# kocvara/Loraine.jl

Hardware: AMD Instinct MI355X
Metric: ms/IP-iteration (Schur assembly + solve), dense SDP n=2000 m=4000 (lower is better)
Workload: dtype f64; 1 GPU; C4 synthetic dense SDP, matrix side 2000, 4000 constraints, kit=0 (assembly + Cholesky + predictor/corrector solves); msz=2000, nvar=4000, seed=20250614, parallelism=1 GPU

## Files before the change

### include/loraine_hip.h

```cpp
#ifndef LORAINE_HIP_H
#define LORAINE_HIP_H

#include <stdint.h>

#ifdef __cplusplus
extern "C" {
#endif

typedef struct lrn_ctx lrn_ctx;

int lrn_create(lrn_ctx** out, int device);
int lrn_destroy(lrn_ctx* ctx);
const char* lrn_last_error(lrn_ctx* ctx);
int lrn_version(void);
int lrn_device_count(void);

int lrn_upload_model(lrn_ctx* ctx, int nlmi, int nvar, const int64_t* msizes,
                     const int64_t* const* AA_colptr, const int64_t* const* AA_rowval,
                     const double* const* AA_nzval,
                     const int64_t* const* B_colptr, const int64_t* const* B_rowval,
                     const double* const* B_nzval,
                     const int64_t* sigmaA, const int64_t* qA,
                     int nlin, const int64_t* Clin_colptr, const int64_t* Clin_rowval,
                     const double* Clin_nzval);
// ... 66 lines not shown
int lrn_comm_allreduce(lrn_ctx* ctx, double* buf, int64_t count, int op);

int lrn_get_timing(lrn_ctx* ctx, const char* key, double* ms);
int64_t lrn_get_count(lrn_ctx* ctx, const char* key);
int lrn_mfma_f64_peak(lrn_ctx* ctx, double* tflops);
int lrn_xcc_probe(lrn_ctx* ctx, int nx, int nz, int hold_us, int32_t* out);
int lrn_hbm_copy_peak(lrn_ctx* ctx, int64_t bytes, double* gbps);

int lrn_dbg_gemm(lrn_ctx* ctx, int transA, int transB, int M, int N, int K, double alpha,
                 const double* A, int lda, const double* B, int ldb, double beta, double* C,
                 int ldc, int flags, int ksplit);
int lrn_dbg_product(lrn_ctx* ctx, int kind, int n, const double* A, const double* Bm, double alpha, double a, int tri,
                    double* out0, double* out1, double* scalar);
int lrn_dbg_gemm_plan(int transA, int transB, int M, int N, int K, int lda, int ldb, double beta, int ldc, int flags,
                      int ksplit, int* out6);
int lrn_dbg_schur_chol_plan(int msz, int nd, int rank, int world, int64_t pcap_hint, const int* opts6, int64_t* out10, int* kb,
                            int* ke, int* weights, double* shares3);
int lrn_dbg_mfma_probe(lrn_ctx* ctx, const double* A16x4, const double* B4x16, double* D16x16);
int lrn_dbg_potrf(lrn_ctx* ctx, int n, double* A, int* info);
int lrn_dbg_potrs(lrn_ctx* ctx, int n, const double* A, const double* b, double* x, int* info);
int lrn_dbg_trsm(lrn_ctx* ctx, int n, int nrhs, int trans, const double* A, double* B, int* info);
int lrn_dbg_svd_jacobi(lrn_ctx* ctx, int n, const double* A, double* U_sigma, double* V,
                       double* sigma, int* sweeps);

#ifdef __cplusplus
}
#endif
#endif
```

### loraine.jl_amd/_capi.py

```python
import ctypes as C
import os
import shutil
import subprocess
import sys

import numpy as np

_HERE = os.path.dirname(os.path.abspath(__file__))
LIB_PATH = os.path.join(_HERE, "libloraine_hip.so")

c_ctx = C.c_void_p
PD = C.POINTER(C.c_double)
PI64 = C.POINTER(C.c_int64)
PI = C.POINTER(C.c_int)
PPD = C.POINTER(C.c_void_p)

SIGNATURES = {
    "lrn_create": (C.c_int, [C.POINTER(c_ctx), C.c_int]),
    "lrn_destroy": (C.c_int, [c_ctx]),
    "lrn_last_error": (C.c_char_p, [c_ctx]),
    "lrn_version": (C.c_int, []),
    "lrn_device_count": (C.c_int, []),
    "lrn_upload_model": (C.c_int, [c_ctx, C.c_int, C.c_int, C.c_void_p, PPD, PPD, PPD, PPD, PPD, PPD,
                                   C.c_void_p, C.c_void_p, C.c_int, C.c_void_p, C.c_void_p, C.c_void_p]),
# ... 47 lines not shown
    "lrn_dbg_get_block": (C.c_int, [c_ctx, C.c_int, C.c_char_p, C.c_void_p, PI]),
    "lrn_dbg_tridiag_eig": (C.c_int, [C.c_int, C.c_void_p, C.c_void_p, C.c_int, C.c_void_p, C.c_double, PD, PI64]),
    "lrn_dbg_eigmin": (C.c_int, [c_ctx, C.c_int, C.c_void_p, PD, PI]),
    "lrn_dbg_lanczos": (C.c_int, [c_ctx, C.c_int, C.c_int, C.c_void_p, C.c_void_p, C.c_void_p, PD, PD, PI]),
    "lrn_get_timing": (C.c_int, [c_ctx, C.c_char_p, PD]),
    "lrn_get_count": (C.c_int64, [c_ctx, C.c_char_p]),
    "lrn_mfma_f64_peak": (C.c_int, [c_ctx, PD]),
    "lrn_hbm_copy_peak": (C.c_int, [c_ctx, C.c_int64, PD]),
    "lrn_xcc_probe": (C.c_int, [c_ctx, C.c_int, C.c_int, C.c_int, C.c_void_p]),
    "lrn_dbg_gemm": (C.c_int, [c_ctx, C.c_int, C.c_int, C.c_int, C.c_int, C.c_int, C.c_double, C.c_void_p,
                               C.c_int, C.c_void_p, C.c_int, C.c_double, C.c_void_p, C.c_int, C.c_int, C.c_int]),
    "lrn_dbg_product": (C.c_int, [c_ctx, C.c_int, C.c_int, C.c_void_p, C.c_void_p, C.c_double, C.c_double, C.c_int,
                                  C.c_void_p, C.c_void_p, PD]),
    "lrn_dbg_gemm_plan": (C.c_int, [C.c_int, C.c_int, C.c_int, C.c_int, C.c_int, C.c_int, C.c_int, C.c_double, C.c_int,
                                    C.c_int, C.c_int, PI]),
    "lrn_dbg_schur_chol_plan": (C.c_int, [C.c_int, C.c_int, C.c_int, C.c_int, C.c_int64, PI, PI64, PI, PI, PI, PD]),
    "lrn_dbg_mfma_probe": (C.c_int, [c_ctx, C.c_void_p, C.c_void_p, C.c_void_p]),
    "lrn_dbg_potrf": (C.c_int, [c_ctx, C.c_int, C.c_void_p, PI]),
    "lrn_dbg_potrs": (C.c_int, [c_ctx, C.c_int, C.c_void_p, C.c_void_p, C.c_void_p, PI]),
    "lrn_dbg_trsm": (C.c_int, [c_ctx, C.c_int, C.c_int, C.c_int, C.c_void_p, C.c_void_p, PI]),
    "lrn_dbg_svd_jacobi": (C.c_int, [c_ctx, C.c_int, C.c_void_p, C.c_void_p, C.c_void_p, C.c_void_p, PI]),
}

GEMM_TRI_LOWER, GEMM_TRI_UPPER, GEMM_OFFDIAG_X2, GEMM_SQUARE, GEMM_KSEG_TRI, GEMM_SMALL_TILE = 1, 2, 4, 8, 16, 32
GEMM_KFROM_N, GEMM_KFROM_M, GEMM_KTO_N, GEMM_KTO_M, GEMM_C_MIRROR, GEMM_DYN_MASKS = 64, 128, 1024, 2048, 4096, 131072

_lib = None


class LoraineHipError(RuntimeError):
# ... 58 lines not shown
```

### loraine.jl_amd/csrc/api.hip

```cpp
#include <cstring>

#include "../../include/loraine_hip.h"
#include "ctx.h"
#include "ops.h"
#include "schur_plan.h"

using namespace lrn;

void lrn_free_model(lrn_ctx* c);
namespace lrn {
void prec_free(lrn_ctx* c);
}

extern "C" {

int lrn_version(void) { return 102; }

int lrn_device_count(void) {
  int n = 0;
  if (hipGetDeviceCount(&n) != hipSuccess) {
    (void)hipGetLastError();
    return 0;
  }
  return n;
// ... 63 lines not shown
  if (!c || !key) return LRN_ERR_ARG;
  if (!strcmp(key, "dense_threshold")) c->opt.dense_threshold = value;
  else if (!strcmp(key, "profile")) c->profile = value != 0.0;
  else if (!strcmp(key, "t_batch")) { c->opt.t_batch = (long)value; for (auto& b : c->lmi) b.t_cap = b.p_cap = 0; }
  else if (!strcmp(key, "p_batch")) { c->opt.p_batch = (long)value; for (auto& b : c->lmi) b.t_cap = b.p_cap = 0; }
  else if (!strcmp(key, "prec_eig")) c->opt.prec_eig = (int)value;
  else if (!strcmp(key, "pivot_boost")) c->opt.pivot_boost = value;
  else if (!strcmp(key, "schur_chol")) c->opt.schur_chol = (int)value;
  else if (!strcmp(key, "schur_plan")) c->opt.schur_plan = (int)value;
  else if (!strcmp(key, "gemm3_ksplit")) c->opt.gemm3_ksplit = (int)value;
  else if (!strcmp(key, "gemm_no_skip")) c->opt.gemm_no_skip = (int)value;
  else if (!strcmp(key, "gemm_dyn_masks")) c->opt.gemm_dyn_masks = (int)value;
  else if (!strcmp(key, "gemm1_diag")) c->opt.gemm1_diag = (int)value;
  else if (!strcmp(key, "gemm_lab")) c->opt.gemm_lab = (int)value & 127;
  else if (!strcmp(key, "gemm3_sched")) c->opt.gemm3_sched = (int)value;
  else if (!strcmp(key, "gemm3_tile")) c->opt.gemm3_tile = (int)value;
  else if (!strcmp(key, "gemm3_strip")) c->opt.gemm3_strip = (int)value;
  else if (!strcmp(key, "gemm3_stagger")) c->opt.gemm3_stagger = (int)value;
  else if (!strcmp(key, "jacobi_wgs")) c->opt.jacobi_wgs = (int)value;
  else if (!strcmp(key, "jacobi_block")) c->opt.jacobi_block = (int)value;
  else if (!strcmp(key, "jacobi_inner")) c->opt.jacobi_inner = (int)value;
  else if (!strcmp(key, "pair_lanes")) c->opt.pair_lanes = (int)value;
  else if (!strcmp(key, "matvec_sparse")) c->opt.matvec_sparse = (int)value;
  else if (!strcmp(key, "prec_dense")) c->opt.prec_dense = (int)value;
  else if (!strcmp(key, "wmw_pattern_min")) c->opt.wmw_pattern_min = std::max(2, (int)value);
  else if (!strcmp(key, "profile_symv")) c->opt.profile_symv = (int)value;
  else if (!strcmp(key, "profile_ops")) c->opt.profile_ops = (int)value;
  else if (!strcmp(key, "matvec_h")) { c->opt.matvec_h = (int)value; c->hop_version = -1; }
  else if (!strcmp(key, "comm_fail_ensure")) lrn::comm_inject_ensure_failure(c);
  else if (!strcmp(key, "pcg_lookahead")) c->opt.pcg_lookahead = std::max(0, std::min(8, (int)value));
// ... 464 lines not shown
    if (flags & GEMM_KSEG_TRI) {
      int ld = 1;
      while ((long)(ld + 1) * (ld + 1) <= K) ++ld;
      g.kseg_ld = ld; g.kseg_cols = ld;
    }
  } else {
    g.sCm = 1; g.sCn = ldc; g.beta = beta;
  }
  GemmPlanInfo info;
  const int rc = gemm_plan_info(g, &info);
  const int v[6] = {info.kernel, info.tile, info.grid_x, info.grid_z, info.dyn_lds, info.slabs};
  for (int i = 0; i < 6; ++i) out6[i] = v[i];
  return rc;
}

int lrn_dbg_schur_chol_plan(int msz, int nd, int rank, int world, int64_t pcap_hint, const int* opts6, int64_t* out10, int* kb,
                            int* ke, int* weights, double* shares3) {
  if (!opts6 || !out10 || !kb || !ke || !weights || !shares3 || msz < 1 || nd < 1 || world < 1 || rank < 0 || rank >= world)
    return LRN_ERR_ARG;
  CholPlanOpts o;
  o.p_batch = opts6[0]; o.gemm3_tile = opts6[1]; o.gemm3_ksplit = opts6[2];
  o.gemm3_sched = opts6[3]; o.gemm3_strip = opts6[4]; o.gemm_no_skip = opts6[5];
  const CholPlan p = plan_chol(msz, nd, rank, world, (long)pcap_hint, o);
  const int64_t v[10] = {p.idle ? -1 : p.c0, p.idle ? -1 : p.c1, p.p_elems, p.ldp, p.P_cap, p.t160 ? 160 : 128,
                         p.ncls,             p.cls[0],           p.cls[1],  p.nslab};
  for (int i = 0; i < 10; ++i) out10[i] = v[i];
  for (int s = 0; s < p.nslab; ++s) { kb[s] = p.kb[s]; ke[s] = p.ke[s]; weights[s] = (int)p.sw.w[s]; }
  shares3[0] = p.gemm1_share; shares3[1] = p.gemm2_share; shares3[2] = p.gemm3_share;
  return LRN_OK;
}
// ... 79 lines not shown
```

### loraine.jl_amd/csrc/ctx.h

```cpp
#pragma once
#include <map>

#include "chol.h"
#include "lrn_common.h"

namespace lrn { struct Prec; struct Comm; }

struct LmiBlock {
  int msz = 0;
  long nent = 0;
  std::vector<int> sigma;
  std::vector<int> ipos;
  std::vector<long> nnz;
  int qA = 0;
  int nd = 0;
  int q_wave = 0;
  int npos_nz = 0;
  long p_cap = 0, t_cap = 0;
  lrn::DBuf ent_ptr;
  lrn::DBuf ent_r, ent_c;
  lrn::DBuf ent_v;
  lrn::DBuf Adense;
  enum DenseRoute { DENSE_SCALAR = 0, DENSE_STREAM, DENSE_TRI };
  DenseRoute dense_route = DENSE_SCALAR;
// ... 47 lines not shown

struct LrnOptions {
  double dense_threshold = -1.0;
  long t_batch = 0, p_batch = 0;
  int prec_eig = 0;
  double pivot_boost = 1e-12;
  int schur_chol = -1;
  int schur_plan = -1;
  int gemm3_ksplit = 0;
  int gemm_dyn_masks = 0;
  int gemm_lab = 0;
  int gemm1_diag = 1;
  int gemm_no_skip = 0;
  int gemm3_sched = 1;
  int gemm3_strip = 1;
  int gemm3_tile = 0;
  int gemm3_stagger = 0;
  int jacobi_inner = 0;
  int jacobi_wgs = 0;
  int jacobi_block = 0;
  int jacobi_cross = 1;
  int prepw_streams = 1;
  int lz_resident = 1;
  int eigmin_pair = 2;
  double jacobi_early = 3e-8;
  bool jacobi_warm = true;
  int shard_passes = 1;
  int prec_inv = -1;
  int nt_mode = 1;
  double ns_l0 = 2e-3;
// ... 144 lines not shown
```

### loraine.jl_amd/csrc/gemm_f64.hip

```cpp
#include "lrn_common.h"

#include <algorithm>
#include <cstdlib>
#include <map>
#include <mutex>
#include <tuple>
#include <type_traits>
#include <utility>
#include <vector>

namespace lrn {

static constexpr int BK = 16;
static constexpr int MAX_KSPLIT = 64;

struct GemmParams {
  GemmDesc d;
  int tilesM, tilesN;
  int kchunk;
  int kcols[MAX_KSPLIT + 1];
  int kcols2[MAX_KSPLIT + 1];
  const int2* tile_list;
  const int2* tile_list2;
  int n1, n2;
  int m_org = 0, n_org = 0;
};

#define MFMA_F64_ROW(lane, r) (((lane) >> 4) + 4 * (r))
#define LRN_MFMA_INPLACE(c, a, b) asm volatile("v_mfma_f64_16x16x4_f64 %0, %1, %2, %0" : "+v"(c) : "v"(a), "v"(b))
#define LRN_MFMA_DRAIN() asm volatile("s_nop 15\n\ts_nop 15\n\ts_nop 15" ::: "memory")

template <int BM, bool KC>
__device__ __forceinline__ int lds_idx(int m, int k) {
  return KC ? (m * (BK + 2) + k) : (k * (BM + 16) + m);
}

template <int BM, int BN, bool AKC, bool BKC, bool KSEG, bool EPI>
__global__ __launch_bounds__(256, 2) void gemm_f64_kernel(GemmParams p) {
  constexpr int TM = BM / 32, TN = BN / 32;
// ... 218 lines not shown
  return bkc ? gemm_f64_kernel<BT, BT, false, true, KSEG, EPI> : gemm_f64_kernel<BT, BT, false, false, KSEG, EPI>;
}
template <int BT>
static GemmFn reg_kernel(const GemmDesc& d, bool epi) {
  if (d.flags & GEMM_KSEG_TRI) return reg_kernel<BT, true, false>(d);
  return epi ? reg_kernel<BT, false, true>(d) : reg_kernel<BT, false, false>(d);
}

template <bool EPI, bool DYN>
__global__ __launch_bounds__(256, 2) void gemm_f64_lds_kernel(GemmParams p) {
  constexpr int BM = 128, BN = 128, TM = 4, TN = 4;
  constexpr int LROW = BM + 16;
  constexpr int LA = BK * LROW;
  __shared__ double lds[2 * 2 * LA];
  const GemmDesc& d = p.d;
  int tm, tn;
  {
    int bid = blockIdx.x, nwg = gridDim.x;
    int q = nwg >> 3, r = nwg & 7, xcd = bid & 7;
    int swz = (xcd < r ? xcd * (q + 1) : r * (q + 1) + (xcd - r) * q) + (bid >> 3);
    if ((d.flags & (GEMM_KFROM_N | GEMM_KFROM_M | GEMM_KTO_N | GEMM_KTO_M)) && r == 0) {
      xcd = (xcd + (int)blockIdx.z) & 7;
      swz = xcd * q + (bid >> 3);
    }
    int2 tt = p.tile_list[swz];
    tm = tt.x;
    tn = tt.y;
  }
  if (tm < 0) return;
  const int bz = blockIdx.z;
  const double* Ag = d.A + (long)bz * d.bA;
  const double* Bg = d.B + (long)bz * d.bB;
  double* __restrict__ Cg = d.C + (long)bz * d.bC;
  const int t = threadIdx.x, lane = t & 63;
  const int w = __builtin_amdgcn_readfirstlane(t >> 6);
  const int wm = w & 1, wn = w >> 1;
  const int m0 = tm * BM, n0 = tn * BN;
  const int lda = (int)d.sAk, ldb = (int)d.sBk;
  const int Me = d.M + (d.M & 1) <= lda ? d.M + (d.M & 1) : d.M;
  const int Ne = d.N + (d.N & 1) <= ldb ? d.N + (d.N & 1) : d.N;
  const unsigned bytesA = (unsigned)(((long)(d.K - 1) * lda + Me) * 8);
  const unsigned bytesB = (unsigned)(((long)(d.K - 1) * ldb + Ne) * 8);
  __amdgpu_buffer_rsrc_t ra = __builtin_amdgcn_make_buffer_rsrc((void*)Ag, 0, bytesA, 0x00020000);
  __amdgpu_buffer_rsrc_t rb = __builtin_amdgcn_make_buffer_rsrc((void*)Bg, 0, bytesB, 0x00020000);
  const int ma = m0 + 2 * lane, nb = n0 + 2 * lane;
// ... 359 lines not shown
#pragma unroll
      for (int r = 0; r < 4; ++r) {
        const int m = m0 + wm * 32 + i * 16 + MFMA_F64_ROW(lane, r);
        const int n = n0 + wn * 32 + j * 16 + fr;
        if (m < d.M && n < d.N) Cg[(long)m * d.sCm + n] = d.alpha * acc[i][j][r];
      }
  if (trace && t == 0) trace[7] = wall_clock64();
}

template <bool FLAT, int TBM, int TBN>
__global__ __launch_bounds__(256, 2) void gemm_f64_kseg_lds_kernel(GemmParams p) {
  constexpr int BM = 32 * TBM, BN = 32 * TBN, TM = TBM, TN = TBN;
  constexpr int LA = BM * BK, LB = BN * BK;
  extern __shared__ double lds[];
  const GemmDesc& d = p.d;
  int tm, tn, ks, bz;
  if (p.n2 >= 0) {
    const int xcd = blockIdx.x & 7, l = blockIdx.x >> 3;
    const int q1 = p.n1 >> 3, q2 = p.n2 >> 3;
    int2 tt;
    if (l < d.ksplit * q1) { ks = l / q1; tt = p.tile_list[xcd * q1 + l % q1]; }
    else { const int l2 = l - d.ksplit * q1; ks = l2 / q2; tt = p.tile_list2[xcd * q2 + l2 % q2]; }
    tm = tt.x;
    tn = tt.y;
    bz = 0;
  } else {
    int bid = blockIdx.x, nwg = gridDim.x;
    int q = nwg >> 3, r = nwg & 7, xcd = bid & 7;
    int swz = (xcd < r ? xcd * (q + 1) : r * (q + 1) + (xcd - r) * q) + (bid >> 3);
    int2 tt = p.tile_list[swz];
    tm = tt.x;
    tn = tt.y;
    ks = blockIdx.z % d.ksplit;
    bz = blockIdx.z / d.ksplit;
  }
  if (tm < 0) return;
  const double* Ag = d.A + (long)bz * d.bA;
  const double* Bg = d.B + (long)bz * d.bB;
  double* __restrict__ Cg = d.C + (long)bz * d.bC + (long)ks * d.sCs;
  const int t = threadIdx.x, lane = t & 63;
  const int w = __builtin_amdgcn_readfirstlane(t >> 6);
  const int wm = w & 1, wn = w >> 1;
  const int m0 = p.m_org + tm * BM, n0 = p.n_org + tn * BN;
  const int lrow = lane >> 3, lpair = lane & 7;
  const double* pa[TBM];
  const double* pb[TBN];
#pragma unroll
  for (int j = 0; j < TBM; ++j) {
    int row = 8 * (w + 4 * j) + lrow;
    int src_pair = lpair ^ ((row >> 1) & 7);
// ... 160 lines not shown
enum GemmKernel : int {
  GK_NONE = 0,
  GK_REG64,
  GK_REG128,
  GK_LDS,
  GK_MID,
  GK_KSEG,
  GK_KFLAT128,
  GK_KFLAT160,
  GK_KFLAT_STRIP,
};

struct TileListKey {
  int tilesM, tilesN, tri, short_sel;
  bool edge_m, edge_n, diag;
  int n;
};

struct GemmPlan {
  GemmKernel kernel;
  int tile_m, tile_n;
  dim3 grid;
  unsigned dyn_lds;
  bool epi;
  int slabs;
  int nlists;
  TileListKey lists[2];
  GemmParams p;
};

static thread_local const char* tls_gemm_error = nullptr;
// ... 22 lines not shown
  const bool tri = d.flags & (GEMM_TRI_LOWER | GEMM_TRI_UPPER);
  return !epi && d.batch == 1 && d.beta == 0.0 && d.sAm == 1 && d.sBn == 1 && d.K >= 64 && d.sCn == 1 && d.sAk >= d.M &&
         d.sBk >= d.N && !(d.flags & ~(GEMM_SMALL_TILE | GEMM_TRI_LOWER | GEMM_TRI_UPPER)) &&
         (!tri || (d.M == d.N && d.ksplit > 1)) && (double)d.K * (double)std::max(d.sAk, d.sBk) * 8.0 < 2.0e9;
}

static bool tile_in_list(const TileListKey& k, int tm, int tn) {
  if (k.tri == GEMM_TRI_LOWER && tn > tm) return false;
  if (k.tri == GEMM_TRI_UPPER && tm > tn) return false;
  const bool shrt = (k.edge_m && tm == k.tilesM - 1) || (k.edge_n && tn == k.tilesN - 1) || (k.diag && tm == tn);
  return !((k.short_sel == 1 && shrt) || (k.short_sel == 2 && !shrt));
}

static TileListKey tile_list_key(int tilesM, int tilesN, int tri, int short_sel = 0, bool edge_m = false, bool edge_n = false,
                                 bool diag = false) {
  TileListKey k{tilesM, tilesN, tri & (GEMM_TRI_LOWER | GEMM_TRI_UPPER), short_sel, edge_m, edge_n, diag, 0};
  if (!k.tri && !short_sel) k.n = tilesM * tilesN;
  else
    for (int tn = 0; tn < tilesN; ++tn)
      for (int tm = 0; tm < tilesM; ++tm) k.n += tile_in_list(k, tm, tn);
  k.n = (k.n + 7) & ~7;
  return k;
}

static const int2* get_tile_list(const TileListKey& k) {
  static std::map<std::tuple<int, int, int>, int2*> cache[16];
  static std::mutex mu;
  std::lock_guard<std::mutex> lock(mu);
  int dev = 0;
  (void)hipGetDevice(&dev);
  auto& cm = cache[dev & 15];
  const std::tuple<int, int, int> key{k.tilesM, k.tilesN, k.tri | k.short_sel << 8 | k.edge_m << 12 | k.edge_n << 13 | k.diag << 14};
  auto it = cm.find(key);
  if (it != cm.end()) return it->second;
  std::vector<int2> v;
  const int GS = 8;
// ... 131 lines not shown
  }
  const bool kseg = d.flags & GEMM_KSEG_TRI;
  if (kseg && kseg_lds_path_ok(d)) return GK_KSEG;
  if (!kseg && !small && lds_path_ok(d)) return GK_LDS;
  if (!kseg && small && mid_path_ok(d, epi)) return GK_MID;
  return small ? GK_REG64 : GK_REG128;
}

static void plan_two_lists(GemmPlan* plan, int tilesM, int tilesN, int tri, bool em, bool en, bool dg) {
  GemmParams& p = plan->p;
  plan->nlists = 2;
  plan->lists[0] = tile_list_key(tilesM, tilesN, tri, 1, em, en, dg);
  plan->lists[1] = tile_list_key(tilesM, tilesN, tri, 2, em, en, dg);
  const bool only_short = plan->lists[0].n == 0;
  if (only_short) plan->lists[0] = plan->lists[1];
  p.n1 = plan->lists[0].n;
  p.n2 = only_short ? 0 : plan->lists[1].n;
}

static int plan_gemm(const GemmDesc& din, GemmPlan* plan, int slabs = 0) {
  *plan = GemmPlan{};
  plan->slabs = slabs > 0 ? slabs : auto_split_factor(din);
  GemmParams& p = plan->p;
  p.d = din;
  GemmDesc& d = p.d;
  if (plan->slabs > 1) {
    d.sCs = (long)din.M * din.N; d.ksplit = plan->slabs; d.beta = 0.0;
    d.flags |= GEMM_SMALL_TILE;
  }
  if (d.M <= 0 || d.N <= 0 || d.batch <= 0) return LRN_OK;
  if (!d.A || !d.B || (!d.C && plan->slabs == 1)) return gemm_fail(LRN_ERR_ARG, "gemm: null A, B or C");
  if (d.ksplit < 1) d.ksplit = 1;
// ... 11 lines not shown
      (!d.blk_w || d.blk_k < 1 || d.blk_k > 16 || (d.blk_k & (d.blk_k - 1)) || d.M % d.blk_k || d.N % d.blk_k ||
       d.ksplit != 1 || d.batch != 1 || kseg || kfrom || d.C2 ||
       (d.flags & (GEMM_SQUARE | GEMM_OFFDIAG_X2 | GEMM_C_PACKED | GEMM_C_MIRROR))))
    return gemm_fail(LRN_ERR_ARG, "gemm: GEMM_SQUARE_BLOCKSUM needs blk_w, blk_k in {1, 2, 4, 8, 16} dividing M and N, one "
                                  "unsplit, unbatched product and no other epilogue");
  if ((d.flags & GEMM_C_PACKED) && (d.pk_off & 15)) return gemm_fail(LRN_ERR_ARG, "gemm: GEMM_C_PACKED needs pk_off % 16 == 0 (block width of the packed layout)");
  if ((d.flags & GEMM_C_PACKED) && (!swapped || d.pk_m <= 0 || d.beta != 0.0)) return gemm_fail(LRN_ERR_ARG, "gemm: (d.flags & GEMM_C_PACKED) && (!swapped || d.pk_m <= 0 || d.beta != 0.0)");
  const bool small = want_small_tile(d, kseg, kfrom);
  const bool big = kflat && (d.flags & GEMM_TILE160);
  const int BMv = small ? 64 : (big ? 160 : 128);
  p.tilesM = (d.M + BMv - 1) / BMv;
  p.tilesN = (d.N + BMv - 1) / BMv;
  if (const int rc = plan_k_ranges(p); rc != LRN_OK) return rc;
  if (d.tile_class >= 4 && !kflat) return gemm_fail(LRN_ERR_ARG, "gemm: tile_class 4 / 5 are for the K-contiguous rank-k update");
  if (d.tile_class != 0 && small) return gemm_fail(LRN_ERR_ARG, "gemm: tile_class needs the 128 tile");
  p.n2 = -1;
  plan->epi = (d.flags & (GEMM_OFFDIAG_X2 | GEMM_SQUARE | GEMM_SQUARE_BLOCKSUM | GEMM_C_PACKED | GEMM_C_MIRROR)) || d.C2;
  plan->tile_m = plan->tile_n = BMv;
  const GemmKernel kernel = choose_kernel(d, small, plan->epi);
  const bool em = (d.M % BMv) != 0, en = (d.N % BMv) != 0, dg = (d.flags & (GEMM_DIAG_LOWER | GEMM_DIAG_UPPER)) != 0;
  if (d.tile_class == 3) {
    if (!kflat || d.batch != 1) return gemm_fail(LRN_ERR_ARG, "gemm: tile_class 3 is for the K-contiguous rank-k update");
    plan_two_lists(plan, p.tilesM, p.tilesN, trif, em, en, dg);
  } else if (d.tile_class == 4 || d.tile_class == 5) {
    const int rem = d.M % 128;
    if (d.batch != 1 || big || d.M != d.N || rem == 0 || rem > 32 || d.M < 288 || trif != GEMM_TRI_UPPER ||
        !(d.flags & GEMM_DIAG_UPPER) || (d.flags & GEMM_NO_SKIP))
      return gemm_fail(LRN_ERR_ARG, "gemm: tile_class 4 needs the symmetric K-contiguous update with M % 128 in (0, 32]");
    const int Mm = d.M - 128 - rem, tmain = Mm / 128;
    if (d.tile_class == 4) {
      d.M = d.N = Mm;
// ... 1 lines not shown
      plan_two_lists(plan, tmain, tmain, GEMM_TRI_UPPER, false, false, true);
    } else {
      d.flags &= ~(GEMM_TRI_LOWER | GEMM_TRI_UPPER | GEMM_DIAG_LOWER | GEMM_DIAG_UPPER);
      p.n_org = Mm;
      p.tilesM = tmain + 2; p.tilesN = 1;
      plan->tile_n = 160;
      plan->nlists = 1;
      plan->lists[0] = tile_list_key(tmain + 2, 1, 0);
    }
  } else {
    plan->nlists = 1;
    plan->lists[0] = tile_list_key(p.tilesM, p.tilesN, trif, d.tile_class, d.tile_class != 0 && em, d.tile_class != 0 && en,
                                   d.tile_class != 0 && dg);
  }
  if (plan->lists[0].n == 0) return LRN_OK;
  if (plan->nlists == 2) {
    const long wgs = 8L * d.ksplit * ((p.n1 >> 3) + (p.n2 >> 3));
    if (wgs > 0x7fffffffL) return gemm_fail(LRN_ERR_ARG, "gemm: grid too large");
    plan->grid = dim3((unsigned)wgs, 1, 1);
  } else {
    plan->grid = dim3(plan->lists[0].n, 1, d.batch * d.ksplit);
    if (plan->grid.z > 65535) return gemm_fail(LRN_ERR_ARG, "gemm: grid.z > 65535");
  }
  if (d.C2 && (d.M != d.N || d.batch != 1 || d.ksplit != 1 || kseg)) return gemm_fail(LRN_ERR_ARG, "gemm: C2 needs a square, unbatched, unsplit product");
  if (kernel == GK_KSEG) plan->dyn_lds = 2 * 2 * 128 * BK * 8;
  else if (kernel > GK_KSEG) plan->dyn_lds = 2 * (plan->tile_m + plan->tile_n) * BK * 8;
  else if (kernel == GK_LDS && (d.flags & (GEMM_LAB_ONE_WG | GEMM_DYN_MASKS)) == GEMM_LAB_ONE_WG) plan->dyn_lds = 24576;
  else if (kernel == GK_MID) {
    p.n1 = (trif ? p.tilesM * (p.tilesM + 1) / 2 : p.tilesM * p.tilesN) * d.ksplit;
    plan->grid = dim3((unsigned)((p.n1 + 7) & ~7), 1, 1);
  }
  plan->kernel = kernel;
  return LRN_OK;
// ... 101 lines not shown
    return LRN_OK;
  }
  if (out) { out->p = din.C; out->stride = 0; out->n = 1; }
  if (!slabs) return LRN_OK;
  const int tri = din.flags != GEMM_TRI_LOWER ? 0 : (std::labs(din.sCm) == 1 ? GEMM_TRI_LOWER : GEMM_TRI_UPPER);
  return reduce_slabs(st, slabs, (long)mn, plan.slabs, din.C, (long)mn, din.beta, tri, din.M);
}

int gemm(hipStream_t st, const GemmDesc& din) { return gemm_maybe_slabs(st, din, nullptr); }
int gemm_slabs(hipStream_t st, const GemmDesc& din, SlabSrc* out) { return gemm_maybe_slabs(st, din, out); }

int gemm_plan_info(const GemmDesc& d, GemmPlanInfo* info) {
  tls_gemm_error = nullptr;
  GemmPlan plan;
  const int rc = plan_gemm(d, &plan);
  *info = GemmPlanInfo{(int)plan.kernel, plan.tile_m, (int)plan.grid.x, (int)plan.grid.z, (int)plan.dyn_lds, plan.slabs};
  return rc;
}

template <bool TRI>
__global__ void reduce_slabs_kernel(const double* __restrict__ slabs, long stride, int nslab,
                                    double* __restrict__ out, long n, double beta, int tri, int ld) {
  long i = (long)blockIdx.x * blockDim.x + threadIdx.x;
  long step = (long)gridDim.x * blockDim.x;
  for (; i < n; i += step) {
    if (TRI) {
      const long r = (i % ld) >> 6, c = (i / ld) >> 6;
      if (tri == GEMM_TRI_LOWER ? r < c : r > c) continue;
    }
    double s = 0.0;
    for (int k = 0; k < nslab; ++k) s += slabs[(long)k * stride + i];
// ... 67 lines not shown
```

### loraine.jl_amd/csrc/lrn_common.h

```cpp
#pragma once
#include <hip/hip_runtime.h>

#include <cstdint>
#include <cstdio>
#include <cstring>
#include <string>
#include <vector>

#define LRN_OK 0
#define LRN_ERR_ARG (-1)
#define LRN_ERR_HIP (-2)
#define LRN_ERR_STATE (-3)
#define LRN_ERR_NOMEM (-4)

typedef double v4f64 __attribute__((ext_vector_type(4)));

namespace lrn {

__host__ __device__ inline int shard_owner(int blk, int world) {
  int r = blk % world;
  return ((blk / world) & 1) ? world - 1 - r : r;
}
__host__ __device__ inline int shard_global_block(int rank, int lb, int world) {
  return lb * world + ((lb & 1) ? world - 1 - rank : rank);
// ... 67 lines not shown
  long sCs = 0;
  int kseg_ld = 0, kseg_cols = 0;
  int pk_m = 0;
  long pk_cstride = 16;
  int pk_off = 0;
  long kflat_cstride = 16;
  const int* kflat_kb = nullptr;
  const int* kflat_ke = nullptr;
  long kflat_total = 0, kflat_diag = 0;
  int kflat_nsd = 0;
  int tile_class = 0;
  unsigned long long* lab_trace = nullptr;
  int kstagger = 0;
  const double* blk_w = nullptr;
  int blk_k = 0;
};

int gemm(hipStream_t st, const GemmDesc& d);
struct SlabSrc {
  const double* p = nullptr;
  long stride = 0;
  int n = 1;
};
__device__ __forceinline__ double slab_sum(const SlabSrc& s, long e) {
  double v = 0.0;
  for (int k = 0; k < s.n; ++k) v += s.p[(long)k * s.stride + e];
  return v;
}
int gemm_slabs(hipStream_t st, const GemmDesc& d, SlabSrc* out);
const char* gemm_last_error();
int reduce_slabs(hipStream_t st, const double* slabs, long stride, int nslab, double* out,
                 long n, double beta, int tri = 0, int ld = 0);
struct GemmPlanInfo { int kernel, tile, grid_x, grid_z, dyn_lds, slabs; };
int gemm_plan_info(const GemmDesc& d, GemmPlanInfo* info);
int mfma_f64_peak(hipStream_t st, double* tflops);
int mfma_f64_probe(hipStream_t st, const double* A16x4, const double* B4x16, double* D16x16);

}
```

### loraine.jl_amd/csrc/schur_dense.hip

```cpp
#include "ops.h"
#include "schur_plan.h"

namespace lrn {

static constexpr int TS = 128;
static constexpr int BK_CHUNK = 16;

__global__ __launch_bounds__(256) void dense_sparse_gather_kernel(
    const long* __restrict__ ptr, const int* __restrict__ er, const int* __restrict__ ec,
    const double* __restrict__ ev, const double* __restrict__ T, int msz, int s0, int ns, int p_lo,
    int p_end, const int* __restrict__ hidx, double* __restrict__ H, int ldh) {
  const int s = blockIdx.y;
  if (s >= ns) return;
  const int pj = p_lo + blockIdx.x * 256 + threadIdx.x;
  if (pj >= p_end) return;
  const double* Ts = T + (long)s * msz * msz;
  double acc = 0.0;
  for (long f = ptr[pj]; f < ptr[pj + 1]; ++f) {
    int p = er[f], q = ec[f];
    int tp = p / TS, tq = q / TS;
    double t;
    if (tp == tq) t = Ts[(long)p + (long)q * msz];
    else if (tp > tq) t = 0.5 * Ts[(long)p + (long)q * msz];
    else t = 0.5 * Ts[(long)q + (long)p * msz];
// ... 133 lines not shown
  return LRN_OK;
}

static int chol_lab12(const LrnOptions& o) {
  return (o.gemm_no_skip ? GEMM_NO_SKIP : 0) | (o.gemm_dyn_masks ? GEMM_DYN_MASKS : 0) | ((o.gemm_lab & 15) << 20);
}
static GemmDesc chol_gemm1(const lrn_ctx* c, const CholPlan& pl, int m, const double* Ad, const double* Ut, double* P, int a,
                           int nbat) {
  const long mm = (long)m * m, off = (long)pl.c0 + (long)pl.c0 * m;
  GemmDesc g1;
  g1.A = Ad + (long)a * mm + off; g1.sAm = 1; g1.sAk = m; g1.bA = mm;
  g1.B = Ut + off; g1.sBk = m; g1.sBn = 1; g1.bB = 0;
  g1.C = P; g1.sCm = pl.ldp; g1.sCn = 1; g1.bC = pl.p_elems;
  g1.M = g1.K = m - pl.c0; g1.N = pl.c1 - pl.c0; g1.batch = nbat;
  g1.flags = GEMM_TRI_LOWER | GEMM_KFROM_N | chol_lab12(c->opt) | (c->opt.gemm1_diag ? GEMM_DIAG_LOWER_Z : 0);
  if (c->opt.gemm_lab & 32) g1.bA = 0;
  if (c->opt.gemm_lab & 16) g1.flags &= ~GEMM_KFROM_N;
  return g1;
}
static GemmDesc chol_gemm2(const lrn_ctx* c, const CholPlan& pl, int m, const double* Ut, const double* P, double* T,
                           long cstride, int a, int nbat) {
  const long off = (long)pl.c0 + (long)pl.c0 * m;
  GemmDesc g2;
  g2.A = Ut + off; g2.sAm = 1; g2.sAk = m; g2.bA = 0;
  g2.B = P; g2.sBk = pl.ldp; g2.sBn = 1; g2.bB = pl.p_elems;
  g2.C = T + (long)a * 16; g2.sCm = 1; g2.sCn = m; g2.bC = 16;
  g2.pk_cstride = cstride;
  g2.M = g2.K = m - pl.c0; g2.N = pl.c1 - pl.c0; g2.batch = nbat;
  g2.flags = GEMM_TRI_LOWER | GEMM_KFROM_M | GEMM_C_PACKED | chol_lab12(c->opt);
  if (c->opt.gemm_lab & 32) g2.bB = 0;
  if (c->opt.gemm_lab & 16) g2.flags &= ~GEMM_KFROM_M;
  g2.pk_m = m;
  g2.pk_off = pl.c0;
  return g2;
}
static GemmDesc chol_gemm3(const lrn_ctx* c, const CholPlan& pl, int m, int nd, const double* T, long cstride, double* slabs) {
  GemmDesc g3;
  g3.A = T; g3.sAm = 16; g3.sAk = 1;
  g3.B = T; g3.sBk = 1; g3.sBn = 16;
  g3.kflat_cstride = cstride;
  g3.C = slabs; g3.sCm = 1; g3.sCn = nd;
  g3.M = nd; g3.N = nd;
  g3.flags = GEMM_TRI_LOWER | GEMM_KFLAT | GEMM_DIAG_LOWER | (c->opt.gemm_no_skip ? GEMM_NO_SKIP : 0) |
             (pl.t160 ? GEMM_TILE160 : 0) | ((c->opt.gemm_lab & 64) ? GEMM_LAB_SAME_CHUNK : 0);
  g3.kflat_total = packed_total_elems(m); g3.kflat_diag = packed_diag_elems(m); g3.kflat_nsd = 1;
  g3.kflat_kb = pl.kb; g3.kflat_ke = pl.ke;
  g3.kstagger = c->opt.gemm3_stagger;
  g3.ksplit = pl.nslab; g3.sCs = (long)nd * nd;
  return g3;
}

static int assemble_dense_chol(lrn_ctx* c, LmiBlock& b, long pcap_hint) {
  const int m = b.msz, nd = b.nd;
  CholPlanOpts po;
  po.p_batch = c->opt.p_batch; po.gemm3_tile = c->opt.gemm3_tile; po.gemm3_ksplit = c->opt.gemm3_ksplit;
  po.gemm3_sched = c->opt.gemm3_sched; po.gemm3_strip = c->opt.gemm3_strip; po.gemm_no_skip = c->opt.gemm_no_skip;
  const CholPlan pl = plan_chol(m, nd, c->rank, c->world, pcap_hint, po);
  c->timing["gemm1_share"] = pl.gemm1_share;
  c->timing["gemm2_share"] = pl.gemm2_share;
  c->timing["gemm3_share"] = pl.gemm3_share;
  const long cstride = 16L * nd;
  LRN_TRY(ensure(c, c->P, (size_t)pl.P_cap * std::max<long>(pl.p_elems, 1) * 8));
// ... 69 lines not shown
    const int s0 = g.first, s1 = g.second, ns = s1 - s0;
    for (int a = s0; a < s1 && via_l; a += (int)P_cap) {
      const int nbat = std::min((int)P_cap, s1 - a);
      double* Lw = c->wchol.as<double>();
      double* Ut = Lw + mm;
      LRN_TRY(ensure(c, c->P2, (size_t)P_cap * mm * 8));
      double* P2 = c->P2.as<double>();
      tic(c);
      GemmDesc g1;
      g1.A = Ad + (long)a * mm; g1.sAm = 1; g1.sAk = m; g1.bA = mm;
      g1.B = Ut; g1.sBk = m; g1.sBn = 1; g1.bB = 0;
      g1.C = P; g1.sCm = m; g1.sCn = 1; g1.bC = mm;
      g1.M = g1.N = g1.K = m; g1.batch = nbat;
      g1.flags = GEMM_TRI_LOWER | GEMM_KFROM_N | (c->opt.gemm_no_skip ? GEMM_NO_SKIP : 0) |
                 (c->opt.gemm_dyn_masks ? GEMM_DYN_MASKS : 0);
      LRN_TRY(gemm(c->stream, g1));
      GemmDesc g2;
      g2.A = Ut; g2.sAm = 1; g2.sAk = m; g2.bA = 0;
      g2.B = P; g2.sBk = m; g2.sBn = 1; g2.bB = mm;
      g2.C = P2; g2.sCm = 1; g2.sCn = m; g2.bC = mm;
      g2.M = g2.N = g2.K = m; g2.batch = nbat;
      g2.flags = GEMM_TRI_LOWER | GEMM_KFROM_M | GEMM_C_MIRROR;
      LRN_TRY(gemm(c->stream, g2));
      toc(c, "gemm1");
      tic(c);
      GemmDesc g3;
      g3.A = Lw; g3.sAm = 1; g3.sAk = m; g3.bA = 0;
      g3.B = P2; g3.sBk = m; g3.sBn = 1; g3.bB = mm;
      g3.C = P; g3.sCm = 1; g3.sCn = m; g3.bC = mm;
      g3.M = g3.N = g3.K = m; g3.batch = nbat;
      g3.flags = GEMM_TRI_LOWER | GEMM_KTO_M;
      LRN_TRY(gemm(c->stream, g3));
      GemmDesc g4;
      g4.A = P; g4.sAm = 1; g4.sAk = m; g4.bA = mm;
      g4.B = Lw; g4.sBk = m; g4.sBn = 1; g4.bB = 0;
      g4.C = T + (long)(a - s0) * mm; g4.sCm = 1; g4.sCn = m; g4.bC = mm;
      g4.M = g4.N = g4.K = m; g4.batch = nbat;
      g4.flags = GEMM_TRI_LOWER | GEMM_OFFDIAG_X2 | GEMM_KTO_N;
      LRN_TRY(gemm(c->stream, g4));
      toc(c, "gemm2");
      c->counts["schur_via_l"] += 1;
    }
    for (int a = s0; a < s1 && !via_l; a += (int)P_cap) {
      const int nbat = std::min((int)P_cap, s1 - a);
      tic(c);
      GemmDesc g1;
      g1.A = Ad + (long)a * mm; g1.sAm = 1; g1.sAk = m; g1.bA = mm;
      g1.B = W; g1.sBk = m; g1.sBn = 1; g1.bB = 0;
      g1.C = P; g1.sCm = m; g1.sCn = 1; g1.bC = mm;
      g1.M = g1.N = g1.K = m; g1.batch = nbat;
      LRN_TRY(gemm(c->stream, g1));
      toc(c, "gemm1");
      tic(c);
// ... 52 lines not shown
```

Baseline: 986.3 ms.

## Unify GEMM workgroup-to-tile dealing and add item-level K-split dealing

Moves the XCD-aware mapping from workgroup to tile into a shared gemm_deal helper used by both GEMM kernels. By default (gemm_deal=2) the K-split rank-k update with batch 1 is dealt as flat (tile, split) items spread evenly across the 8 XCDs. Previously whole tile runs per split were assigned, which left the XCDs unevenly loaded. This is meant to cut tail imbalance in the Schur assembly GEMMs. In exchange it adds more index arithmetic per workgroup, including a small loop, and changes L2 locality per XCD.

```diff
diff --git a/include/loraine_hip.h b/include/loraine_hip.h
--- a/include/loraine_hip.h
+++ b/include/loraine_hip.h
@@ -104,6 +104,8 @@
                     double* out0, double* out1, double* scalar);
 int lrn_dbg_gemm_plan(int transA, int transB, int M, int N, int K, int lda, int ldb, double beta, int ldc, int flags,
                       int ksplit, int* out6);
+int lrn_dbg_gemm_deal(int mode, int r1, int r2, int batch, int ksplit, int64_t flat0, int64_t count, int* out4,
+                      int64_t* total);
 int lrn_dbg_schur_chol_plan(int msz, int nd, int rank, int world, int64_t pcap_hint, const int* opts6, int64_t* out10, int* kb,
                             int* ke, int* weights, double* shares3);
 int lrn_dbg_mfma_probe(lrn_ctx* ctx, const double* A16x4, const double* B4x16, double* D16x16);
diff --git a/loraine.jl_amd/_capi.py b/loraine.jl_amd/_capi.py
--- a/loraine.jl_amd/_capi.py
+++ b/loraine.jl_amd/_capi.py
@@ -85,6 +85,7 @@
                                   C.c_void_p, C.c_void_p, PD]),
     "lrn_dbg_gemm_plan": (C.c_int, [C.c_int, C.c_int, C.c_int, C.c_int, C.c_int, C.c_int, C.c_int, C.c_double, C.c_int,
                                     C.c_int, C.c_int, PI]),
+    "lrn_dbg_gemm_deal": (C.c_int, [C.c_int, C.c_int, C.c_int, C.c_int, C.c_int, C.c_int64, C.c_int64, PI, PI64]),
     "lrn_dbg_schur_chol_plan": (C.c_int, [C.c_int, C.c_int, C.c_int, C.c_int, C.c_int64, PI, PI64, PI, PI, PI, PD]),
     "lrn_dbg_mfma_probe": (C.c_int, [c_ctx, C.c_void_p, C.c_void_p, C.c_void_p]),
     "lrn_dbg_potrf": (C.c_int, [c_ctx, C.c_int, C.c_void_p, PI]),
diff --git a/loraine.jl_amd/csrc/api.hip b/loraine.jl_amd/csrc/api.hip
--- a/loraine.jl_amd/csrc/api.hip
+++ b/loraine.jl_amd/csrc/api.hip
@@ -2,6 +2,7 @@
 
 #include "../../include/loraine_hip.h"
 #include "ctx.h"
+#include "gemm_deal.h"
 #include "ops.h"
 #include "schur_plan.h"
 
@@ -101,6 +102,7 @@
   else if (!strcmp(key, "gemm1_diag")) c->opt.gemm1_diag = (int)value;
   else if (!strcmp(key, "gemm_lab")) c->opt.gemm_lab = (int)value & 127;
   else if (!strcmp(key, "gemm3_sched")) c->opt.gemm3_sched = (int)value;
+  else if (!strcmp(key, "gemm_deal")) c->opt.gemm_deal = (int)value & 3;
   else if (!strcmp(key, "gemm3_tile")) c->opt.gemm3_tile = (int)value;
   else if (!strcmp(key, "gemm3_strip")) c->opt.gemm3_strip = (int)value;
   else if (!strcmp(key, "gemm3_stagger")) c->opt.gemm3_stagger = (int)value;
@@ -595,6 +597,23 @@
   return rc;
 }
 
+int lrn_dbg_gemm_deal(int mode, int r1, int r2, int batch, int ksplit, int64_t flat0, int64_t count, int* out4, int64_t* total) {
+  if (mode < GEMM_DEAL_RUNS || mode > GEMM_DEAL_ITEMS || r1 < 1 || r2 < 0 || batch < 1 || ksplit < 1 || flat0 < 0 || count < 0 ||
+      (count > 0 && !out4))
+    return LRN_ERR_ARG;
+  if ((mode == GEMM_DEAL_TWO_RUNS || mode == GEMM_DEAL_ITEMS) && batch != 1) return LRN_ERR_ARG;
+  if (mode == GEMM_DEAL_MATRIX && ksplit != 1) return LRN_ERR_ARG;
+  if (r2 > 0 && mode != GEMM_DEAL_TWO_RUNS && mode != GEMM_DEAL_ITEMS) return LRN_ERR_ARG;
+  const long n = gemm_deal_flat(mode, r1, r2, batch, ksplit);
+  if (n > 0x7fffffffL || flat0 + count > n) return LRN_ERR_ARG;
+  if (total) *total = n;
+  for (int64_t i = 0; i < count; ++i) {
+    const GemmDealItem it = gemm_deal(mode, r1, r2, batch, ksplit, (unsigned)(flat0 + i));
+    out4[4 * i] = it.list; out4[4 * i + 1] = it.entry; out4[4 * i + 2] = it.batch; out4[4 * i + 3] = it.split;
+  }
+  return LRN_OK;
+}
+
 int lrn_dbg_schur_chol_plan(int msz, int nd, int rank, int world, int64_t pcap_hint, const int* opts6, int64_t* out10, int* kb,
                             int* ke, int* weights, double* shares3) {
   if (!opts6 || !out10 || !kb || !ke || !weights || !shares3 || msz < 1 || nd < 1 || world < 1 || rank < 0 || rank >= world)
diff --git a/loraine.jl_amd/csrc/ctx.h b/loraine.jl_amd/csrc/ctx.h
--- a/loraine.jl_amd/csrc/ctx.h
+++ b/loraine.jl_amd/csrc/ctx.h
@@ -85,6 +85,7 @@
   int gemm_no_skip = 0;
   int gemm3_sched = 1;
   int gemm3_strip = 1;
+  int gemm_deal = 2;
   int gemm3_tile = 0;
   int gemm3_stagger = 0;
   int jacobi_inner = 0;
diff --git a/loraine.jl_amd/csrc/gemm_deal.h b/loraine.jl_amd/csrc/gemm_deal.h
--- /dev/null
+++ b/loraine.jl_amd/csrc/gemm_deal.h
@@ -0,0 +1,90 @@
+#pragma once
+
+#if defined(__HIPCC__) || defined(__CUDACC__)
+#define LRN_DEAL_HD __host__ __device__
+#else
+#define LRN_DEAL_HD
+#endif
+
+namespace lrn {
+
+enum GemmDealMode : int {
+  GEMM_DEAL_RUNS = 0,
+  GEMM_DEAL_RUNS_ROT = 1,
+  GEMM_DEAL_TWO_RUNS = 2,
+  GEMM_DEAL_MATRIX = 3,
+  GEMM_DEAL_ITEMS = 4,
+};
+
+struct GemmDealItem {
+  int list;
+  int entry;
+  int batch;
+  int split;
+};
+
+LRN_DEAL_HD inline int gemm_deal_pad8(int r) { return (r + 7) & ~7; }
+
+LRN_DEAL_HD inline long gemm_deal_flat(int mode, int r1, int r2, int batch, int ksplit) {
+  switch (mode) {
+    case GEMM_DEAL_TWO_RUNS: return (long)ksplit * (gemm_deal_pad8(r1) + gemm_deal_pad8(r2));
+    case GEMM_DEAL_ITEMS: return ((long)ksplit * ((long)r1 + r2) + 7) & ~7L;
+    default: return (long)gemm_deal_pad8(r1) * batch * ksplit;
+  }
+}
+
+LRN_DEAL_HD inline GemmDealItem gemm_deal(int mode, int r1, int r2, int batch, int ksplit, unsigned flat) {
+  const GemmDealItem padding{-1, 0, 0, 0};
+  const unsigned x = flat & 7u, l = flat >> 3;
+  const unsigned n1 = (unsigned)gemm_deal_pad8(r1), n2 = (unsigned)gemm_deal_pad8(r2);
+  switch (mode) {
+    case GEMM_DEAL_MATRIX: {
+      const unsigned full = (unsigned)(batch >> 3) * 8u * n1;
+      if (flat < full) {
+        const unsigned g = l / n1, t = l - g * n1;
+        if (t >= (unsigned)r1) return padding;
+        return GemmDealItem{0, (int)t, (int)(8u * g + x), 0};
+      }
+    }
+    [[fallthrough]];
+    case GEMM_DEAL_RUNS:
+    case GEMM_DEAL_RUNS_ROT: {
+      const unsigned z = flat / n1, bid = flat - z * n1;
+      const unsigned xr = mode == GEMM_DEAL_RUNS ? x : ((x + z) & 7u);
+      const unsigned e = xr * (n1 >> 3) + (bid >> 3);
+      if (e >= (unsigned)r1) return padding;
+      const unsigned b = z / (unsigned)ksplit;
+      return GemmDealItem{0, (int)e, (int)b, (int)(z - b * (unsigned)ksplit)};
+    }
+    case GEMM_DEAL_TWO_RUNS: {
+      const unsigned q1 = n1 >> 3, q2 = n2 >> 3;
+      if (l < (unsigned)ksplit * q1) {
+        const unsigned s = l / q1, e = x * q1 + (l - s * q1);
+        if (e >= (unsigned)r1) return padding;
+        return GemmDealItem{0, (int)e, 0, (int)s};
+      }
+      if (q2 == 0) return padding;
+      const unsigned l2 = l - (unsigned)ksplit * q1, s = l2 / q2, e = x * q2 + (l2 - s * q2);
+      if (s >= (unsigned)ksplit || e >= (unsigned)r2) return padding;
+      return GemmDealItem{1, (int)e, 0, (int)s};
+    }
+    case GEMM_DEAL_ITEMS: {
+      const unsigned i1 = (unsigned)ksplit * (unsigned)r1, b1 = i1 >> 3, m1 = i1 & 7u;
+      const unsigned c1 = b1 + (x < m1 ? 1u : 0u);
+      if (l < c1) {
+        const unsigned i = x * b1 + (x < m1 ? x : m1) + l, s = i / (unsigned)r1;
+        return GemmDealItem{0, (int)(i - s * (unsigned)r1), 0, (int)s};
+      }
+      const unsigned i2 = (unsigned)ksplit * (unsigned)r2, b2 = i2 >> 3, m2 = i2 & 7u;
+      unsigned before = 0;
+      for (unsigned y = 0; y < x; ++y) before += ((y - m1) & 7u) < m2 ? 1u : 0u;
+      const unsigned c2 = b2 + (((x - m1) & 7u) < m2 ? 1u : 0u), la = l - c1;
+      if (la >= c2) return padding;
+      const unsigned i = x * b2 + before + la, s = i / (unsigned)r2;
+      return GemmDealItem{1, (int)(i - s * (unsigned)r2), 0, (int)s};
+    }
+  }
+  return padding;
+}
+
+}
diff --git a/loraine.jl_amd/csrc/gemm_f64.hip b/loraine.jl_amd/csrc/gemm_f64.hip
--- a/loraine.jl_amd/csrc/gemm_f64.hip
+++ b/loraine.jl_amd/csrc/gemm_f64.hip
@@ -1,4 +1,5 @@
 #include "lrn_common.h"
+#include "gemm_deal.h"
 
 #include <algorithm>
 #include <cstdlib>
@@ -22,7 +23,9 @@
   int kcols2[MAX_KSPLIT + 1];
   const int2* tile_list;
   const int2* tile_list2;
-  int n1, n2;
+  int n1;
+  int r1 = 0, r2 = 0;
+  int deal = 0;
   int m_org = 0, n_org = 0;
 };
 
@@ -271,21 +274,12 @@
   constexpr int LA = BK * LROW;
   __shared__ double lds[2 * 2 * LA];
   const GemmDesc& d = p.d;
-  int tm, tn;
-  {
-    int bid = blockIdx.x, nwg = gridDim.x;
-    int q = nwg >> 3, r = nwg & 7, xcd = bid & 7;
-    int swz = (xcd < r ? xcd * (q + 1) : r * (q + 1) + (xcd - r) * q) + (bid >> 3);
-    if ((d.flags & (GEMM_KFROM_N | GEMM_KFROM_M | GEMM_KTO_N | GEMM_KTO_M)) && r == 0) {
-      xcd = (xcd + (int)blockIdx.z) & 7;
-      swz = xcd * q + (bid >> 3);
-    }
-    int2 tt = p.tile_list[swz];
-    tm = tt.x;
-    tn = tt.y;
-  }
+  const GemmDealItem it = gemm_deal(p.deal, p.r1, 0, d.batch, 1, blockIdx.x + gridDim.x * blockIdx.z);
+  if (it.list < 0) return;
+  const int2 tt = p.tile_list[it.entry];
+  const int tm = tt.x, tn = tt.y;
   if (tm < 0) return;
-  const int bz = blockIdx.z;
+  const int bz = it.batch;
   const double* Ag = d.A + (long)bz * d.bA;
   const double* Bg = d.B + (long)bz * d.bB;
   double* __restrict__ Cg = d.C + (long)bz * d.bC;
@@ -675,26 +669,10 @@
   constexpr int LA = BM * BK, LB = BN * BK;
   extern __shared__ double lds[];
   const GemmDesc& d = p.d;
-  int tm, tn, ks, bz;
-  if (p.n2 >= 0) {
-    const int xcd = blockIdx.x & 7, l = blockIdx.x >> 3;
-    const int q1 = p.n1 >> 3, q2 = p.n2 >> 3;
-    int2 tt;
-    if (l < d.ksplit * q1) { ks = l / q1; tt = p.tile_list[xcd * q1 + l % q1]; }
-    else { const int l2 = l - d.ksplit * q1; ks = l2 / q2; tt = p.tile_list2[xcd * q2 + l2 % q2]; }
-    tm = tt.x;
-    tn = tt.y;
-    bz = 0;
-  } else {
-    int bid = blockIdx.x, nwg = gridDim.x;
-    int q = nwg >> 3, r = nwg & 7, xcd = bid & 7;
-    int swz = (xcd < r ? xcd * (q + 1) : r * (q + 1) + (xcd - r) * q) + (bid >> 3);
-    int2 tt = p.tile_list[swz];
-    tm = tt.x;
-    tn = tt.y;
-    ks = blockIdx.z % d.ksplit;
-    bz = blockIdx.z / d.ksplit;
-  }
+  const GemmDealItem it = gemm_deal(p.deal, p.r1, p.r2, d.batch, d.ksplit, blockIdx.x + gridDim.x * blockIdx.z);
+  if (it.list < 0) return;
+  const int2 tt = (it.list ? p.tile_list2 : p.tile_list)[it.entry];
+  const int tm = tt.x, tn = tt.y, ks = it.split, bz = it.batch;
   if (tm < 0) return;
   const double* Ag = d.A + (long)bz * d.bA;
   const double* Bg = d.B + (long)bz * d.bB;
@@ -885,7 +863,7 @@
 struct TileListKey {
   int tilesM, tilesN, tri, short_sel;
   bool edge_m, edge_n, diag;
-  int n;
+  int real, n;
 };
 
 struct GemmPlan {
@@ -938,12 +916,12 @@
 
 static TileListKey tile_list_key(int tilesM, int tilesN, int tri, int short_sel = 0, bool edge_m = false, bool edge_n = false,
                                  bool diag = false) {
-  TileListKey k{tilesM, tilesN, tri & (GEMM_TRI_LOWER | GEMM_TRI_UPPER), short_sel, edge_m, edge_n, diag, 0};
-  if (!k.tri && !short_sel) k.n = tilesM * tilesN;
+  TileListKey k{tilesM, tilesN, tri & (GEMM_TRI_LOWER | GEMM_TRI_UPPER), short_sel, edge_m, edge_n, diag, 0, 0};
+  if (!k.tri && !short_sel) k.real = tilesM * tilesN;
   else
     for (int tn = 0; tn < tilesN; ++tn)
-      for (int tm = 0; tm < tilesM; ++tm) k.n += tile_in_list(k, tm, tn);
-  k.n = (k.n + 7) & ~7;
+      for (int tm = 0; tm < tilesM; ++tm) k.real += tile_in_list(k, tm, tn);
+  k.n = gemm_deal_pad8(k.real);
   return k;
 }
 
@@ -1105,8 +1083,7 @@
   plan->lists[1] = tile_list_key(tilesM, tilesN, tri, 2, em, en, dg);
   const bool only_short = plan->lists[0].n == 0;
   if (only_short) plan->lists[0] = plan->lists[1];
-  p.n1 = plan->lists[0].n;
-  p.n2 = only_short ? 0 : plan->lists[1].n;
+  p.r2 = only_short ? 0 : plan->lists[1].real;
 }
 
 static int plan_gemm(const GemmDesc& din, GemmPlan* plan, int slabs = 0) {
@@ -1148,7 +1125,6 @@
   if (const int rc = plan_k_ranges(p); rc != LRN_OK) return rc;
   if (d.tile_class >= 4 && !kflat) return gemm_fail(LRN_ERR_ARG, "gemm: tile_class 4 / 5 are for the K-contiguous rank-k update");
   if (d.tile_class != 0 && small) return gemm_fail(LRN_ERR_ARG, "gemm: tile_class needs the 128 tile");
-  p.n2 = -1;
   plan->epi = (d.flags & (GEMM_OFFDIAG_X2 | GEMM_SQUARE | GEMM_SQUARE_BLOCKSUM | GEMM_C_PACKED | GEMM_C_MIRROR)) || d.C2;
   plan->tile_m = plan->tile_n = BMv;
   const GemmKernel kernel = choose_kernel(d, small, plan->epi);
@@ -1180,9 +1156,14 @@
                                    d.tile_class != 0 && dg);
   }
   if (plan->lists[0].n == 0) return LRN_OK;
-  if (plan->nlists == 2) {
-    const long wgs = 8L * d.ksplit * ((p.n1 >> 3) + (p.n2 >> 3));
-    if (wgs > 0x7fffffffL) return gemm_fail(LRN_ERR_ARG, "gemm: grid too large");
+  p.r1 = plan->lists[0].real;
+  if (kflat && d.batch == 1 && (d.deal & 2)) p.deal = GEMM_DEAL_ITEMS;
+  else if (plan->nlists == 2) p.deal = GEMM_DEAL_TWO_RUNS;
+  else if (kernel == GK_LDS && kfrom) p.deal = (d.deal & 1) && d.batch >= 8 ? GEMM_DEAL_MATRIX : GEMM_DEAL_RUNS_ROT;
+  else p.deal = GEMM_DEAL_RUNS;
+  const long wgs = gemm_deal_flat(p.deal, p.r1, p.r2, d.batch, d.ksplit);
+  if (wgs > 0x7fffffffL) return gemm_fail(LRN_ERR_ARG, "gemm: grid too large");
+  if (p.deal == GEMM_DEAL_ITEMS || p.deal == GEMM_DEAL_TWO_RUNS) {
     plan->grid = dim3((unsigned)wgs, 1, 1);
   } else {
     plan->grid = dim3(plan->lists[0].n, 1, d.batch * d.ksplit);
@@ -1314,7 +1295,7 @@
   tls_gemm_error = nullptr;
   GemmPlan plan;
   const int rc = plan_gemm(d, &plan);
-  *info = GemmPlanInfo{(int)plan.kernel, plan.tile_m, (int)plan.grid.x, (int)plan.grid.z, (int)plan.dyn_lds, plan.slabs};
+  *info = GemmPlanInfo{(int)plan.kernel, plan.tile_m, (int)plan.grid.x, (int)plan.grid.z, (int)plan.dyn_lds, plan.slabs, plan.p.deal};
   return rc;
 }
 
diff --git a/loraine.jl_amd/csrc/lrn_common.h b/loraine.jl_amd/csrc/lrn_common.h
--- a/loraine.jl_amd/csrc/lrn_common.h
+++ b/loraine.jl_amd/csrc/lrn_common.h
@@ -105,6 +105,7 @@
   int kstagger = 0;
   const double* blk_w = nullptr;
   int blk_k = 0;
+  int deal = 0;
 };
 
 int gemm(hipStream_t st, const GemmDesc& d);
@@ -122,7 +123,7 @@
 const char* gemm_last_error();
 int reduce_slabs(hipStream_t st, const double* slabs, long stride, int nslab, double* out,
                  long n, double beta, int tri = 0, int ld = 0);
-struct GemmPlanInfo { int kernel, tile, grid_x, grid_z, dyn_lds, slabs; };
+struct GemmPlanInfo { int kernel, tile, grid_x, grid_z, dyn_lds, slabs, deal; };
 int gemm_plan_info(const GemmDesc& d, GemmPlanInfo* info);
 int mfma_f64_peak(hipStream_t st, double* tflops);
 int mfma_f64_probe(hipStream_t st, const double* A16x4, const double* B4x16, double* D16x16);
diff --git a/loraine.jl_amd/csrc/schur_dense.hip b/loraine.jl_amd/csrc/schur_dense.hip
--- a/loraine.jl_amd/csrc/schur_dense.hip
+++ b/loraine.jl_amd/csrc/schur_dense.hip
@@ -171,6 +171,7 @@
   g1.C = P; g1.sCm = pl.ldp; g1.sCn = 1; g1.bC = pl.p_elems;
   g1.M = g1.K = m - pl.c0; g1.N = pl.c1 - pl.c0; g1.batch = nbat;
   g1.flags = GEMM_TRI_LOWER | GEMM_KFROM_N | chol_lab12(c->opt) | (c->opt.gemm1_diag ? GEMM_DIAG_LOWER_Z : 0);
+  g1.deal = c->opt.gemm_deal;
   if (c->opt.gemm_lab & 32) g1.bA = 0;
   if (c->opt.gemm_lab & 16) g1.flags &= ~GEMM_KFROM_N;
   return g1;
@@ -185,6 +186,7 @@
   g2.pk_cstride = cstride;
   g2.M = g2.K = m - pl.c0; g2.N = pl.c1 - pl.c0; g2.batch = nbat;
   g2.flags = GEMM_TRI_LOWER | GEMM_KFROM_M | GEMM_C_PACKED | chol_lab12(c->opt);
+  g2.deal = c->opt.gemm_deal;
   if (c->opt.gemm_lab & 32) g2.bB = 0;
   if (c->opt.gemm_lab & 16) g2.flags &= ~GEMM_KFROM_M;
   g2.pk_m = m;
@@ -203,6 +205,7 @@
   g3.kflat_total = packed_total_elems(m); g3.kflat_diag = packed_diag_elems(m); g3.kflat_nsd = 1;
   g3.kflat_kb = pl.kb; g3.kflat_ke = pl.ke;
   g3.kstagger = c->opt.gemm3_stagger;
+  g3.deal = c->opt.gemm_deal;
   g3.ksplit = pl.nslab; g3.sCs = (long)nd * nd;
   return g3;
 }
@@ -302,6 +305,7 @@
       g1.M = g1.N = g1.K = m; g1.batch = nbat;
       g1.flags = GEMM_TRI_LOWER | GEMM_KFROM_N | (c->opt.gemm_no_skip ? GEMM_NO_SKIP : 0) |
                  (c->opt.gemm_dyn_masks ? GEMM_DYN_MASKS : 0);
+      g1.deal = c->opt.gemm_deal;
       LRN_TRY(gemm(c->stream, g1));
       GemmDesc g2;
       g2.A = Ut; g2.sAm = 1; g2.sAk = m; g2.bA = 0;
@@ -309,6 +313,7 @@
       g2.C = P2; g2.sCm = 1; g2.sCn = m; g2.bC = mm;
       g2.M = g2.N = g2.K = m; g2.batch = nbat;
       g2.flags = GEMM_TRI_LOWER | GEMM_KFROM_M | GEMM_C_MIRROR;
+      g2.deal = c->opt.gemm_deal;
       LRN_TRY(gemm(c->stream, g2));
       toc(c, "gemm1");
       tic(c);
@@ -318,6 +323,7 @@
       g3.C = P; g3.sCm = 1; g3.sCn = m; g3.bC = mm;
       g3.M = g3.N = g3.K = m; g3.batch = nbat;
       g3.flags = GEMM_TRI_LOWER | GEMM_KTO_M;
+      g3.deal = c->opt.gemm_deal;
       LRN_TRY(gemm(c->stream, g3));
       GemmDesc g4;
       g4.A = P; g4.sAm = 1; g4.sAk = m; g4.bA = mm;
@@ -325,6 +331,7 @@
       g4.C = T + (long)(a - s0) * mm; g4.sCm = 1; g4.sCn = m; g4.bC = mm;
       g4.M = g4.N = g4.K = m; g4.batch = nbat;
       g4.flags = GEMM_TRI_LOWER | GEMM_OFFDIAG_X2 | GEMM_KTO_N;
+      g4.deal = c->opt.gemm_deal;
       LRN_TRY(gemm(c->stream, g4));
       toc(c, "gemm2");
       c->counts["schur_via_l"] += 1;
```

Measured after the change: 978.9 ms (median of 6 runs). Within noise of the previous version (-0.8%).
